# homenc/HElib

Hardware: NVIDIA H100
Metric: ctxt_mults_per_s (higher is better)
Workload: dtype u64

## Files before the change

helib_b200/csrc/hb_device_v1.cuh:

```cuda
#pragma once
#include <utility>
#include "hb_device.cuh"

#define HB1_RS 17
#define HB1_BS 273

__device__ __forceinline__ void hb_group_sync(int group, int nthreads) {
#ifdef HB_SIM
  cusim::bar_sync(1 + group, nthreads);
#else
  asm volatile("bar.sync %0, %1;" ::"r"(1 + group), "r"(nthreads) : "memory");
#endif
}

__device__ __forceinline__ void hb1_mac128(u64& hi, u64& lo, u64 a, u64 b) {
#ifdef HB_SIM
  hb_mac128(hi, lo, a, b);
#else
  asm("{\n\t.reg .u64 pl, ph;\n\t"
      "mul.lo.u64 pl, %2, %3;\n\t"
      "mul.hi.u64 ph, %2, %3;\n\t"
      "add.cc.u64 %0, %0, pl;\n\t"
      "addc.u64 %1, %1, ph;\n\t}"
      : "+l"(lo), "+l"(hi)
// ... 137 lines not shown
  asm volatile("cp.async.ca.shared.global [%0], [%1], 8;" ::"r"(sa), "l"(src) : "memory");
#endif
}
__device__ __forceinline__ void hb1_cp_commit() {
#ifndef HB_SIM
  asm volatile("cp.async.commit_group;" ::: "memory");
#endif
}
template <int N> __device__ __forceinline__ void hb1_cp_wait() {
#ifndef HB_SIM
  asm volatile("cp.async.wait_group %0;" ::"n"(N) : "memory");
#endif
}

#define HB1_STAGE (16 * HB1_BS + 8)

struct Hb1Unit { int rowi, ug, it; };
__device__ __forceinline__ Hb1Unit hb1_unit_next(Hb1Unit x, int G, int nitems) {
  if (++x.it == nitems) { x.it = 0; if (++x.ug == G) { x.ug = 0; ++x.rowi; } }
  return x;
}
__device__ __forceinline__ Hb1Unit hb1_unit(long u, int G, int nitems) {
  Hb1Unit x;
  const unsigned per_row = (unsigned)(G * nitems), uu = (unsigned)u;
  x.rowi = (int)(uu / per_row);
  const int rem = (int)(uu - (unsigned)x.rowi * per_row);
  x.ug = rem / nitems;
  x.it = rem - x.ug * nitems;
  return x;
}

template <bool SP>
__global__ void __launch_bounds__(256, 2) k1_fwd_blk(const HbPrimeDev* __restrict__ primes, const HB_GRID_CONSTANT Hb1BlkJob J) {
  HB_SMEM_DECL
  u64* S = HB_SMEM;
  u64* O = S + 2 * HB1_STAGE;
  ulonglong2* TW1 = (ulonglong2*)(O + 16 * 256);
  const int tid = threadIdx.x;
  const int n1 = J.logN - 8;
  const int G = 1 << (n1 - 4);
  const long U = (long)J.rows.n * G * J.nitems;
  const long ubeg = U * blockIdx.x / gridDim.x, uend = U * (blockIdx.x + 1) / gridDim.x;
  if (ubeg >= uend) return;
  const int blk1 = tid >> 4, lo = tid & 15;
  const int hi = tid >> 4, blk2 = tid & 15;
  const unsigned hrev = hb1_brev4(hi);
  const bool epi1 = J.epi == 1, epi3 = J.epi == 3, lazy = J.lazy != 0;
  const int own = blk1 * HB1_BS + lo;
  Hb1TwPtr tw1;
  tw1.p[0] = TW1 + blk1 * 16; tw1.p[1] = tw1.p[0] + 1; tw1.p[2] = tw1.p[0] + 3; tw1.p[3] = tw1.p[0] + 7;

  auto src_ptr = [&](const Hb1Unit& x) {
    const unsigned b = hb_brev((x.ug << 4) + blk1, n1);
    return J.src[x.it] + ((size_t)J.rows.prime[x.rowi] << J.logN) + ((size_t)b << 8) + lo;
  };
  Hb1Unit cur = hb1_unit(ubeg, G, J.nitems);
  {
    const u64* src = src_ptr(cur);
    hb1_unroll<16>([&](auto r) { hb1_cp8(S + own + HB1_RS * r, src + 16 * r); });
  }
  hb1_cp_commit();
  int key = -1, buf = 0;
  u64 q = 0, sc = 0, sc_s = 0;
  Hb1Mod M; M.nq = 0; M.qb = 0; M.qb2 = 0; M.qt = 0; M.qsh = 0;
  Hb1TwReg tw2;
  for (long u = ubeg; u < uend; u++, buf ^= 1) {
    if (cur.rowi * G + cur.ug != key) {
      key = cur.rowi * G + cur.ug;
      const HbPrimeDev P = primes[J.rows.prime[cur.rowi]];
      q = P.q; M.nq = P.nq; M.qb = P.qb; M.qb2 = P.qb + P.qb; M.qt = P.qt; M.qsh = P.qsh;
      sc = J.scal[cur.rowi]; sc_s = J.scal_s[cur.rowi];
      const unsigned b1 = hb_brev((cur.ug << 4) + blk1, n1), b2 = hb_brev((cur.ug << 4) + blk2, n1);
      if (lo < 15) {
        int e = lo, k = e >= 7 ? 3 : (e >= 3 ? 2 : (e >= 1 ? 1 : 0));
        int g = e - ((1 << k) - 1);
        TW1[blk1 * 16 + e] = P.fw[((size_t)1 << (n1 + k)) + ((size_t)b1 << k) + g];
      }
      tw2.load([&](int k, int g) { return P.fw[((size_t)1 << (n1 + 4 + k)) + ((size_t)b2 << (4 + k)) + ((size_t)hi << k) + g]; });
      __syncthreads();
    }
    u64* Sb = S + buf * HB1_STAGE;
    const size_t doff = ((size_t)J.rows.prime[cur.rowi] << J.logN) + (cur.ug << 4) + blk2;
    u64* dst = J.dst[cur.it] + doff;
    const bool epi = epi1 || (epi3 && sc != 0);
    u64* old = epi3 ? J.dst2[cur.it] + doff : dst;
    if (epi) {
      hb1_unroll<16>([&](auto l) { hb1_cp8(O + l * 256 + tid, old + ((size_t)((hb1_brev4(l) << 4) | hrev) << n1)); });
    }
    hb1_cp_commit();
    Hb1Unit nxt = cur;
    if (u + 1 < uend) {
      nxt = hb1_unit_next(cur, G, J.nitems);
      const u64* src = src_ptr(nxt);
      u64* Sn = S + (buf ^ 1) * HB1_STAGE;
      hb1_unroll<16>([&](auto r) { hb1_cp8(Sn + own + HB1_RS * r, src + 16 * r); });
    }
    hb1_cp_commit();
    hb1_cp_wait<2>();
    u64 a[16];
    hb1_unroll<16>([&](auto r) { a[r] = Sb[own + HB1_RS * r]; });
    hb1_r16_fwd<SP>(a, tw1, M);
    hb1_unroll<16>([&](auto r) { Sb[own + HB1_RS * r] = a[r]; });
    __syncthreads();
    hb1_unroll<16>([&](auto l) { a[l] = Sb[blk2 * HB1_BS + HB1_RS * hi + l]; });
    hb1_r16_fwd<SP>(a, tw2, M);
    hb1_cp_wait<1>();
    hb1_unroll<16>([&](auto l) {
      const size_t o = (size_t)((hb1_brev4(l) << 4) | hrev) << n1;
      if (epi) {
        u64 v = hb1_shoup4<SP>(O[l * 256 + tid] - a[l] + (M.qb2 + M.qb), sc, sc_s, M);
        if (!lazy) v = hb1_canon4(v, q);
        old[o] = v;
      }
      if (!epi1) dst[o] = lazy ? a[l] : hb1_canon_fwd(a[l], q, M.qb);
    });
    __syncthreads();
    cur = nxt;
  }
  hb1_cp_wait<0>();
}

template <bool SP>
__global__ void __launch_bounds__(256, 1) k1_fwd_blk_tensor(const HbPrimeDev* __restrict__ primes, const HB_GRID_CONSTANT Hb1BlkJob J) {
  HB_SMEM_DECL
  u64* S = HB_SMEM;
  u64* O = S + 2 * HB1_STAGE;
  ulonglong2* TW1 = (ulonglong2*)(O + 16 * 256);
  u64* V = (u64*)(TW1 + 256);
  const int tid = threadIdx.x;
  const int n1 = J.logN - 8;
  const int G = 1 << (n1 - 4);
  const long U = (long)J.rows.n * G * J.nitems;
  const long ubeg = U * blockIdx.x / gridDim.x, uend = U * (blockIdx.x + 1) / gridDim.x;
  if (ubeg >= uend) return;
  const int blk1 = tid >> 4, lo = tid & 15;
  const int hi = tid >> 4, blk2 = tid & 15;
  const unsigned hrev = hb1_brev4(hi);
  const int own = blk1 * HB1_BS + lo;
  u64* const Vt = V + tid;
  Hb1TwPtr tw1;
  tw1.p[0] = TW1 + blk1 * 16; tw1.p[1] = tw1.p[0] + 1; tw1.p[2] = tw1.p[0] + 3; tw1.p[3] = tw1.p[0] + 7;

  auto prefetch = [&](u64* Sn, const Hb1Unit& x, int k) {
    const unsigned b = hb_brev((x.ug << 4) + blk1, n1);
    const u64* src = J.src[4 * x.it + k] + ((size_t)J.rows.prime[x.rowi] << J.logN) + ((size_t)b << 8) + lo;
    hb1_unroll<16>([&](auto r) { hb1_cp8(Sn + own + HB1_RS * r, src + 16 * r); });
  };
  Hb1Unit cur = hb1_unit(ubeg, G, J.nitems);
  prefetch(S, cur, 0);
  hb1_cp_commit();
  int key = -1;
  u64 q = 0, sc = 0, sc_s = 0, c64 = 0, c64_s = 0, one_s = 0;
  Hb1Mod M; M.nq = 0; M.qb = 0; M.qb2 = 0; M.qt = 0; M.qsh = 0;
  Hb1TwReg tw2;
  for (long u = ubeg; u < uend; u++) {
    if (cur.rowi * G + cur.ug != key) {
      key = cur.rowi * G + cur.ug;
      const HbPrimeDev P = primes[J.rows.prime[cur.rowi]];
      q = P.q; M.nq = P.nq; M.qb = P.qb; M.qb2 = P.qb + P.qb; M.qt = P.qt; M.qsh = P.qsh;
      c64 = P.c64; c64_s = P.c64_s; one_s = P.one_s;
      sc = J.scal[cur.rowi]; sc_s = J.scal_s[cur.rowi];
      const unsigned b1 = hb_brev((cur.ug << 4) + blk1, n1), b2 = hb_brev((cur.ug << 4) + blk2, n1);
      if (lo < 15) {
        int e = lo, k = e >= 7 ? 3 : (e >= 3 ? 2 : (e >= 1 ? 1 : 0));
        int g = e - ((1 << k) - 1);
        TW1[blk1 * 16 + e] = P.fw[((size_t)1 << (n1 + k)) + ((size_t)b1 << k) + g];
      }
      tw2.load([&](int k, int g) { return P.fw[((size_t)1 << (n1 + 4 + k)) + ((size_t)b2 << (4 + k)) + ((size_t)hi << k) + g]; });
      __syncthreads();
    }
    const size_t doff = ((size_t)J.rows.prime[cur.rowi] << J.logN) + (cur.ug << 4) + blk2;
    u64* const* dst = J.dst + 4 * cur.it;
    const bool more = u + 1 < uend;
    const Hb1Unit nxt = more ? hb1_unit_next(cur, G, J.nitems) : cur;
#pragma unroll 1
    for (int k = 0; k < 4; k++) {
      u64* Sb = S + (k & 1) * HB1_STAGE;
      const u64* old = dst[k] + doff;
      hb1_unroll<16>([&](auto l) { hb1_cp8(O + l * 256 + tid, old + ((size_t)((hb1_brev4(l) << 4) | hrev) << n1)); });
      hb1_cp_commit();
      if (k < 3) prefetch(S + ((k + 1) & 1) * HB1_STAGE, cur, k + 1);
      else if (more) prefetch(S, nxt, 0);
      hb1_cp_commit();
      hb1_cp_wait<2>();
      u64 a[16];
      hb1_unroll<16>([&](auto r) { a[r] = Sb[own + HB1_RS * r]; });
      hb1_r16_fwd<SP>(a, tw1, M);
      hb1_unroll<16>([&](auto r) { Sb[own + HB1_RS * r] = a[r]; });
      __syncthreads();
      hb1_unroll<16>([&](auto l) { a[l] = Sb[blk2 * HB1_BS + HB1_RS * hi + l]; });
      hb1_r16_fwd<SP>(a, tw2, M);
      hb1_cp_wait<1>();
      hb1_unroll<16>([&](auto l) {
        a[l] = hb1_shoup4<SP>(O[l * 256 + tid] - a[l] + (M.qb2 + M.qb), sc, sc_s, M);
      });
      if (k < 2) {
        hb1_unroll<16>([&](auto l) { Vt[k * 4096 + l * 256] = a[l]; });
      } else if (k == 2) {
        hb1_unroll<16>([&](auto l) {
          const size_t o = doff + ((size_t)((hb1_brev4(l) << 4) | hrev) << n1);
          const u64 x0 = Vt[l * 256], x1 = Vt[4096 + l * 256], v = a[l];
          dst[0][o] = hb_reduce128(__umul64hi(x0, v), x0 * v, q, c64, c64_s, one_s);
          Vt[2 * 4096 + l * 256] = hb_reduce128(__umul64hi(x1, v), x1 * v, q, c64, c64_s, one_s);
        });
      } else {
        hb1_unroll<16>([&](auto l) {
          const size_t o = doff + ((size_t)((hb1_brev4(l) << 4) | hrev) << n1);
          const u64 x0 = Vt[l * 256], x1 = Vt[4096 + l * 256], v = a[l];
          u64 h = 0, w = Vt[2 * 4096 + l * 256];
          hb1_mac128(h, w, x0, v);
          dst[1][o] = hb_reduce128(h, w, q, c64, c64_s, one_s);
          dst[2][o] = hb_reduce128(__umul64hi(x1, v), x1 * v, q, c64, c64_s, one_s);
          dst[3][o] = v;
        });
      }
      __syncthreads();
    }
    cur = nxt;
  }
  hb1_cp_wait<0>();
}

template <bool SP>
__global__ void __launch_bounds__(256, 2) k1_inv_blk(const HbPrimeDev* __restrict__ primes, const HB_GRID_CONSTANT Hb1BlkJob J) {
  HB_SMEM_DECL
  u64* S = HB_SMEM;
  ulonglong2* TW1 = (ulonglong2*)(S + 2 * HB1_STAGE);
  const int tid = threadIdx.x;
  const int n1 = J.logN - 8;
  const int G = 1 << (n1 - 4);
  const long U = (long)J.rows.n * G * J.nitems;
  const long ubeg = U * blockIdx.x / gridDim.x, uend = U * (blockIdx.x + 1) / gridDim.x;
  if (ubeg >= uend) return;
  const int blk1 = tid >> 4, lo = tid & 15;
  const int hi = tid >> 4, blk2 = tid & 15;
  const unsigned hrev = hb1_brev4(hi);
  Hb1TwPtr tw1;
  tw1.p[0] = TW1 + blk1 * 16; tw1.p[1] = tw1.p[0] + 1; tw1.p[2] = tw1.p[0] + 3; tw1.p[3] = tw1.p[0] + 7;
  const int own = blk2 * HB1_BS + HB1_RS * hi;
  auto src_ptr = [&](const Hb1Unit& x) {
    return J.src[x.it] + ((size_t)J.rows.prime[x.rowi] << J.logN) + (x.ug << 4) + blk2;
  };
  Hb1Unit cur = hb1_unit(ubeg, G, J.nitems);
  {
    const u64* src = src_ptr(cur);
    hb1_unroll<16>([&](auto l) { hb1_cp8(S + own + l, src + ((size_t)((hb1_brev4(l) << 4) | hrev) << n1)); });
  }
  hb1_cp_commit();
  int key = -1, buf = 0;
  u64 q = 0;
  Hb1Mod M; M.nq = 0; M.qb = 0; M.qb2 = 0; M.qt = 0; M.qsh = 0;
  unsigned b1 = 0;
  Hb1TwReg tw2;
  for (long u = ubeg; u < uend; u++, buf ^= 1) {
    if (cur.rowi * G + cur.ug != key) {
      key = cur.rowi * G + cur.ug;
      const HbPrimeDev P = primes[J.rows.prime[cur.rowi]];
      q = P.q; M.nq = P.nq; M.qb = P.qb; M.qb2 = P.qb + P.qb; M.qt = P.qt; M.qsh = P.qsh;
      b1 = hb_brev((cur.ug << 4) + blk1, n1);
      const unsigned b2 = hb_brev((cur.ug << 4) + blk2, n1);
      if (lo < 15) {
        int e = lo, k = e >= 7 ? 3 : (e >= 3 ? 2 : (e >= 1 ? 1 : 0));
        int g = e - ((1 << k) - 1);
        TW1[blk1 * 16 + e] = P.iw[((size_t)1 << (n1 + k)) + ((size_t)b1 << k) + g];
      }
      tw2.load([&](int k, int g) { return P.iw[((size_t)1 << (n1 + 4 + k)) + ((size_t)b2 << (4 + k)) + ((size_t)hi << k) + g]; });
      __syncthreads();
    }
    u64* Sb = S + buf * HB1_STAGE;
    Hb1Unit nxt = cur;
    if (u + 1 < uend) {
      nxt = hb1_unit_next(cur, G, J.nitems);
      const u64* src = src_ptr(nxt);
      u64* Sn = S + (buf ^ 1) * HB1_STAGE;
      hb1_unroll<16>([&](auto l) { hb1_cp8(Sn + own + l, src + ((size_t)((hb1_brev4(l) << 4) | hrev) << n1)); });
    }
    hb1_cp_commit();
    hb1_cp_wait<1>();
    u64 a[16];
    hb1_unroll<16>([&](auto l) { a[l] = Sb[own + l]; });
    hb1_r16_inv<SP>(a, tw2, M);
    hb1_unroll<16>([&](auto l) { Sb[own + l] = a[l]; });
    __syncthreads();
    hb1_unroll<16>([&](auto r) { a[r] = Sb[blk1 * HB1_BS + HB1_RS * r + lo]; });
    hb1_r16_inv<SP>(a, tw1, M);
    u64* dst = J.dst[cur.it] + ((size_t)J.rows.prime[cur.rowi] << J.logN) + ((size_t)b1 << 8) + lo;
    hb1_unroll<16>([&](auto r) { dst[16 * r] = J.epi == 2 ? a[r] : hb1_canon_inv(a[r], q); });
    __syncthreads();
    cur = nxt;
  }
  hb1_cp_wait<0>();
}

struct Hb1ColsJob {
  int logN;
  HbRows rows;
  int nitems;
  const u64* src[HB_MAXB];
  u64* dst[HB_MAXB];
  int has_scal, npeers;
  u64 scal[HB_MAXROWS], scal_s[HB_MAXROWS];
  u64* peer[8][HB_MAXB];
};

// ... 316 lines not shown
```

helib_b200/csrc/hb_engine.cu:

```cuda
#include "hb_device.cuh"
#include "hb_device_v1.cuh"
#include "hb_device_v2.cuh"
#include "hb_device_gen.cuh"
#include "hb_device_prg.cuh"

#include <algorithm>
#include <cmath>
#include <cstdarg>
#include <cstdio>
#include <cstdlib>
#include <cstring>
#include <map>
#include <set>
#include <string>
#include <vector>

#include "../../include/helib_b200.h"

typedef unsigned __int128 u128;

static size_t blk_tensor_smem() {
  return (2 * HB1_STAGE + 16 * 256 + 3 * 16 * 256) * sizeof(u64) + 256 * sizeof(ulonglong2);
}

static thread_local char g_err[512] = "";
static thread_local int g_chunk = HB_MAXB;
static int hb_fail(int code, const char* fmt, ...) {
  va_list ap; va_start(ap, fmt); vsnprintf(g_err, sizeof(g_err), fmt, ap); va_end(ap);
  return code;
}
#define HB_CUDA(x) do { cudaError_t e_ = (x); if (e_ != cudaSuccess) return hb_fail(HB_ERR_CUDA, "%s failed: %s (%s:%d)", #x, cudaGetErrorString(e_), __FILE__, __LINE__); } while (0)
#define HB_TRY(x) do { int r_ = (x); if (r_ != HB_OK) return r_; } while (0)

static inline u64 h_mulmod(u64 a, u64 b, u64 q) { return (u64)((u128)a * b % q); }
static inline u64 h_powmod(u64 a, u64 e, u64 q) {
  u64 r = 1 % q; a %= q;
  while (e) { if (e & 1) r = h_mulmod(r, a, q); a = h_mulmod(a, a, q); e >>= 1; }
  return r;
// ... 200 lines not shown
      u64 qi = c->q[i];
      HbPrimeDev& P = c->h_primes[i];
      memset(&P, 0, sizeof(P));
      P.q = qi; P.c64 = (u64)(((u128)1 << 64) % qi); P.c64_s = h_shoup(P.c64, qi); P.one_s = (u64)(((u128)1 << 64) / qi);
      P.nq = 0 - qi; P.qb = 4 * qi;
      { int sh = 0; u64 t = qi - 1; while ((t & 1) == 0) { t >>= 1; sh++; }
        if (sh >= 32 && t < (1ULL << 32)) { P.qt = (unsigned)t; P.qsh = (unsigned)(sh - 32); } }
    }
    HB_TRY(ctx_alloc(c, (void**)&c->d_primes, sizeof(HbPrimeDev) * nprimes));
    HB_CUDA(cudaMemcpy(c->d_primes, c->h_primes.data(), sizeof(HbPrimeDev) * nprimes, cudaMemcpyHostToDevice));
    HB_TRY(ctx_alloc(c, (void**)&c->d_stats, 4 * sizeof(u64)));
    HB_CUDA(cudaMemset(c->d_stats, 0, 4 * sizeof(u64)));
#ifndef HB_SIM
    HB_CUDA(cudaFuncSetAttribute(k_fwd_blk, cudaFuncAttributeMaxDynamicSharedMemorySize, 64 * 1024));
    HB_CUDA(cudaFuncSetAttribute(k_inv_blk, cudaFuncAttributeMaxDynamicSharedMemorySize, 64 * 1024));
    HB_CUDA(cudaFuncSetAttribute(k1_fwd_blk<true>, cudaFuncAttributeMaxDynamicSharedMemorySize, 112 * 1024));
  HB_CUDA(cudaFuncSetAttribute(k1_fwd_blk<false>, cudaFuncAttributeMaxDynamicSharedMemorySize, 112 * 1024));
    HB_CUDA(cudaFuncSetAttribute(k1_inv_blk<true>, cudaFuncAttributeMaxDynamicSharedMemorySize, 80 * 1024));
  HB_CUDA(cudaFuncSetAttribute(k1_inv_blk<false>, cudaFuncAttributeMaxDynamicSharedMemorySize, 80 * 1024));
    HB_CUDA(cudaFuncSetAttribute(k2_fwd_blk<true>, cudaFuncAttributeMaxDynamicSharedMemorySize, (int)HB2_SMEM_BYTES));
    HB_CUDA(cudaFuncSetAttribute(k2_fwd_blk<false>, cudaFuncAttributeMaxDynamicSharedMemorySize, (int)HB2_SMEM_BYTES));
    HB_CUDA(cudaFuncSetAttribute(k2_inv_blk<true>, cudaFuncAttributeMaxDynamicSharedMemorySize, (int)HB2_SMEM_BYTES));
    HB_CUDA(cudaFuncSetAttribute(k2_inv_blk<false>, cudaFuncAttributeMaxDynamicSharedMemorySize, (int)HB2_SMEM_BYTES));
#endif
    HB_TRY(gen_init(c, psi));
    *out = c;
    return HB_OK;
  }
  std::vector<ulonglong2> tw((size_t)nprimes * 2 * N);
  std::vector<u64> pw(N);
  std::vector<unsigned> brev(N);
  for (size_t k = 0; k < N; k++) { unsigned r = 0; for (int b = 0; b < c->logN; b++) if (k >> b & 1) r |= 1u << (c->logN - 1 - b); brev[k] = r; }
  HB_TRY(ctx_alloc(c, (void**)&c->d_tw, tw.size() * sizeof(ulonglong2)));
  c->h_primes.resize(nprimes);
// ... 22 lines not shown
  HB_CUDA(cudaMemcpy(c->d_primes, c->h_primes.data(), sizeof(HbPrimeDev) * nprimes, cudaMemcpyHostToDevice));
  HB_TRY(ctx_alloc(c, (void**)&c->d_stats, 4 * sizeof(u64)));
  HB_CUDA(cudaMemset(c->d_stats, 0, 4 * sizeof(u64)));
#ifndef HB_SIM
  HB_CUDA(cudaFuncSetAttribute(k_conv, cudaFuncAttributeMaxDynamicSharedMemorySize, (int)c->max_smem + 1024));
  HB_CUDA(cudaFuncSetAttribute(k_fwd_blk, cudaFuncAttributeMaxDynamicSharedMemorySize, 64 * 1024));
  HB_CUDA(cudaFuncSetAttribute(k_inv_blk, cudaFuncAttributeMaxDynamicSharedMemorySize, 64 * 1024));
  HB_CUDA(cudaFuncSetAttribute(k2_fwd_blk<true>, cudaFuncAttributeMaxDynamicSharedMemorySize, (int)HB2_SMEM_BYTES));
  HB_CUDA(cudaFuncSetAttribute(k2_fwd_blk<false>, cudaFuncAttributeMaxDynamicSharedMemorySize, (int)HB2_SMEM_BYTES));
  HB_CUDA(cudaFuncSetAttribute(k2_inv_blk<true>, cudaFuncAttributeMaxDynamicSharedMemorySize, (int)HB2_SMEM_BYTES));
  HB_CUDA(cudaFuncSetAttribute(k2_inv_blk<false>, cudaFuncAttributeMaxDynamicSharedMemorySize, (int)HB2_SMEM_BYTES));
  HB_CUDA(cudaFuncSetAttribute(k1_conv1<true>, cudaFuncAttributeMaxDynamicSharedMemorySize, 128 * 1024));
  HB_CUDA(cudaFuncSetAttribute(k1_conv1<false>, cudaFuncAttributeMaxDynamicSharedMemorySize, 128 * 1024));
  HB_CUDA(cudaFuncSetAttribute(k1_conv<true>, cudaFuncAttributeMaxDynamicSharedMemorySize, 227 * 1024));
  HB_CUDA(cudaFuncSetAttribute(k1_conv<false>, cudaFuncAttributeMaxDynamicSharedMemorySize, 227 * 1024));
  HB_CUDA(cudaFuncSetAttribute(k1_fwd_blk<true>, cudaFuncAttributeMaxDynamicSharedMemorySize, 112 * 1024));
  HB_CUDA(cudaFuncSetAttribute(k1_fwd_blk<false>, cudaFuncAttributeMaxDynamicSharedMemorySize, 112 * 1024));
  HB_CUDA(cudaFuncSetAttribute(k1_inv_blk<true>, cudaFuncAttributeMaxDynamicSharedMemorySize, 80 * 1024));
  HB_CUDA(cudaFuncSetAttribute(k1_inv_blk<false>, cudaFuncAttributeMaxDynamicSharedMemorySize, 80 * 1024));
  HB_CUDA(cudaFuncSetAttribute(k1_fwd_blk_tensor<true>, cudaFuncAttributeMaxDynamicSharedMemorySize, (int)blk_tensor_smem()));
  HB_CUDA(cudaFuncSetAttribute(k1_fwd_blk_tensor<false>, cudaFuncAttributeMaxDynamicSharedMemorySize, (int)blk_tensor_smem()));
#endif
  *out = c;
  return HB_OK;
}

extern "C" void hb_ctx_destroy(hb_ctx* c) {
  if (!c) return;
  if (c->stream) cudaStreamSynchronize(c->stream);
  for (auto& kv : c->convs) { cudaFree(kv.second.blob); cudaFree(kv.second.d); }
  for (hb_poly* p : c->pool) { cudaFree(p->d); delete p; }
  cudaFree(c->pw.d_cube_to_poly); cudaFree(c->pw.d_short_to_long); cudaFree(c->pw.cube); cudaFree(c->pw.rows);
  cudaFree(c->d_frac); cudaFree(c->d_z); cudaFree(c->d_max); cudaFree(c->d_bcast);
  cudaFree(c->gen.d_rep); cudaFree(c->gen.d_irep); cudaFree(c->gen.d_gp); cudaFree(c->gen.d_primes_cyc); cudaFree(c->gen.d_primes_cyc2); cudaFree(c->gen.tab);
  cudaFree(c->gen.d_W);
  cudaFree(c->gen.w0); cudaFree(c->gen.w1); cudaFree(c->gen.wt); cudaFree(c->gen.cA); cudaFree(c->gen.cB);
// ... 437 lines not shown
static bool v1_cols_ok(hb_ctx* c) { return !c->force_v0 && c->log_blk == 8 && c->logN - 8 == 8; }
static int pick_item_groups(hb_ctx* c, long ctas_per_item_group, int nitems) {
  int best = 1; double best_eff = -1;
  for (int z = 1; z <= nitems; z++) {
    long ctas = ctas_per_item_group * z;
    long waves = (ctas + c->resident_ctas - 1) / c->resident_ctas;
    int per = (nitems + z - 1) / z;
    double eff = (double)ctas / (double)(waves * c->resident_ctas) * ((double)nitems / (double)(per * z));
    if (eff > best_eff + 0.02) { best_eff = eff; best = z; }
  }
  return best;
}
static int launch_blk_v1(hb_ctx* c, int dir, const u64* const* src, u64* const* dst, int nitems, const int32_t* idx, int n,
                         int epi, const u64* scal, int lazy = 0, u64* const* dst2 = nullptr) {
  const int n1 = c->logN - 8;
  const size_t smem = (2 * HB1_STAGE + (dir > 0 ? 16 * 256 : 0)) * sizeof(u64) + 256 * sizeof(ulonglong2);
  for (int r0 = 0; r0 < n; r0 += HB_MAXROWS) {
    int nr = std::min(HB_MAXROWS, n - r0);
    Hb1BlkJob J; memset(&J, 0, sizeof(J));
    J.logN = c->logN; J.epi = epi; J.lazy = lazy;
    if (dir < 0) J.epi = v1_cols_ok(c) ? 2 : 0;
    fill_rows(J.rows, idx + r0, nr);
    for (int i = 0; i < nr; i++) if (scal) { J.scal[i] = scal[r0 + i]; J.scal_s[i] = h_shoup(scal[r0 + i], c->q[idx[r0 + i]]); }
    J.nitems = nitems;
    for (int i = 0; i < nitems; i++) { J.src[i] = src[i]; J.dst[i] = dst[i]; if (dst2) J.dst2[i] = dst2[i]; }
    long units = (long)nr * nitems << (n1 - 4);
    dim3 grid((unsigned)std::min<long>(units, c->resident_ctas));
    pre_launch(c);
    const bool sp = all_special(c);
    if (dir > 0) { if (sp) HB_LAUNCH(k1_fwd_blk<true>, grid, dim3(256), smem, c->stream, c->d_primes, J); else HB_LAUNCH(k1_fwd_blk<false>, grid, dim3(256), smem, c->stream, c->d_primes, J); HB_TRY(post_launch(c, epi == 1 ? "k1_fwd_blk_subscale" : (epi == 3 ? "k1_fwd_blk_digits" : "k1_fwd_blk"), (u64)(epi == 1 ? 3 : 2) * nr * nitems * c->N * 8)); }
    else { if (sp) HB_LAUNCH(k1_inv_blk<true>, grid, dim3(256), smem, c->stream, c->d_primes, J); else HB_LAUNCH(k1_inv_blk<false>, grid, dim3(256), smem, c->stream, c->d_primes, J); HB_TRY(post_launch(c, "k1_inv_blk", (u64)2 * nr * nitems * c->N * 8)); }
  }
  return HB_OK;
}
static int launch_blk_tensor_v1(hb_ctx* c, const u64* const* src, u64* const* dst, int nitems, const int32_t* idx, int n, const u64* scal) {
  const int n1 = c->logN - 8;
  for (int r0 = 0; r0 < n; r0 += HB_MAXROWS) {
    int nr = std::min(HB_MAXROWS, n - r0);
    Hb1BlkJob J; memset(&J, 0, sizeof(J));
    J.logN = c->logN; J.epi = 1; J.lazy = 1;
    fill_rows(J.rows, idx + r0, nr);
    for (int i = 0; i < nr; i++) { J.scal[i] = scal[r0 + i]; J.scal_s[i] = h_shoup(scal[r0 + i], c->q[idx[r0 + i]]); }
    J.nitems = nitems;
    for (int i = 0; i < 4 * nitems; i++) { J.src[i] = src[i]; J.dst[i] = dst[i]; }
    long units = (long)nr * nitems << (n1 - 4);
    dim3 grid((unsigned)std::min<long>(units, std::max(1, c->resident_ctas / 2)));
    pre_launch(c);
    if (all_special(c)) HB_LAUNCH(k1_fwd_blk_tensor<true>, grid, dim3(256), blk_tensor_smem(), c->stream, c->d_primes, J);
    else HB_LAUNCH(k1_fwd_blk_tensor<false>, grid, dim3(256), blk_tensor_smem(), c->stream, c->d_primes, J);
    HB_TRY(post_launch(c, "k1_fwd_blk_tensor", (u64)12 * nr * nitems * c->N * 8));
  }
  return HB_OK;
}

#define HB_TMAP_SLAB 512
#ifndef HB_SIM
typedef CUresult (*hb_encode_tiled_fn)(CUtensorMap*, CUtensorMapDataType, cuuint32_t, void*, const cuuint64_t*, const cuuint64_t*,
                                       const cuuint32_t*, const cuuint32_t*, CUtensorMapInterleave, CUtensorMapSwizzle,
                                       CUtensorMapL2promotion, CUtensorMapFloatOOBfill);
static hb_encode_tiled_fn hb_encode_tiled() {
  static hb_encode_tiled_fn fn = [] {
    void* p = nullptr; cudaDriverEntryPointQueryResult qr;
    if (cudaGetDriverEntryPoint("cuTensorMapEncodeTiled", &p, cudaEnableDefault, &qr) != cudaSuccess || qr != cudaDriverEntryPointSuccess) p = nullptr;
    return (hb_encode_tiled_fn)p;
// ... 1959 lines not shown
```

Before: 2948.

## Deepen NTT block kernel pipelines to triple-buffered inputs with prefetched epilogue operands

The forward and inverse blocked NTT kernels move from double to triple buffering of staged input tiles, and the forward kernel also double-buffers the epilogue's old-value tile so it is fetched one unit ahead. The tensor kernel prefetches its per-part epilogue operands after the previous part's stores instead of right before use. To fit the extra shared memory, launch bounds drop to one CTA per SM and the grid is halved, which trades occupancy for deeper async-copy overlap. The change also adds compile-time ablation switches and a standalone microbenchmark.

```diff
diff --git a/bench_micro/ubench_blk.cu b/bench_micro/ubench_blk.cu
--- /dev/null
+++ b/bench_micro/ubench_blk.cu
@@ -0,0 +1,106 @@
+#include <cstdio>
+#include <cstdlib>
+#include <cstring>
+#include <vector>
+#include <cuda_runtime.h>
+#include "../helib_b200/csrc/hb_device_v1.cuh"
+
+#define CK(x) do { cudaError_t e_ = (x); if (e_ != cudaSuccess) { fprintf(stderr, "%s: %s (line %d)\n", #x, cudaGetErrorString(e_), __LINE__); exit(1); } } while (0)
+
+typedef unsigned __int128 u128;
+static const int LOGN = 16, NPR = 30, NPOLY = 192;
+static const size_t N = (size_t)1 << LOGN;
+
+static u64 rng_state = 0x9E3779B97F4A7C15ULL;
+static u64 rnd() { rng_state ^= rng_state << 13; rng_state ^= rng_state >> 7; rng_state ^= rng_state << 17; return rng_state; }
+
+__global__ void fill_random(u64* p, size_t n, u64 q, u64 seed) {
+  for (size_t i = blockIdx.x * (size_t)blockDim.x + threadIdx.x; i < n; i += (size_t)gridDim.x * blockDim.x) {
+    u64 x = (i + 1) * 0x9E3779B97F4A7C15ULL ^ seed;
+    x ^= x >> 29; x *= 0xBF58476D1CE4E5B9ULL; x ^= x >> 32;
+    p[i] = x % q;
+  }
+}
+
+struct Primes { HbPrimeDev* d; std::vector<u64> q; };
+static Primes make_primes(bool sp, ulonglong2* tw) {
+  Primes P; std::vector<HbPrimeDev> h(NPR);
+  std::vector<ulonglong2> t(2 * N);
+  for (int i = 0; i < NPR; i++) {
+    const u64 qt = (1ULL << 27) - 2 * i - 1;
+    const u64 q = sp ? (qt << 33) + 1 : (1ULL << 60) - (((u64)i + 1) << 20) - 1;
+    P.q.push_back(q);
+    HbPrimeDev& H = h[i]; memset(&H, 0, sizeof(H));
+    H.q = q; H.c64 = (u64)(((u128)1 << 64) % q); H.c64_s = (u64)(((u128)H.c64 << 64) / q); H.one_s = (u64)(((u128)1 << 64) / q);
+    H.nq = 0 - q; H.qb = 4 * q;
+    if (sp) { H.qt = (unsigned)qt; H.qsh = 1; }
+    for (size_t k = 0; k < 2 * N; k++) { u64 w = rnd() % q; t[k] = make_ulonglong2(w, (u64)(((u128)w << 64) / q)); }
+    CK(cudaMemcpy(tw + (size_t)i * 2 * N, t.data(), t.size() * sizeof(ulonglong2), cudaMemcpyHostToDevice));
+    H.fw = tw + (size_t)i * 2 * N; H.iw = H.fw + N;
+  }
+  CK(cudaMalloc(&P.d, sizeof(HbPrimeDev) * NPR));
+  CK(cudaMemcpy(P.d, h.data(), sizeof(HbPrimeDev) * NPR, cudaMemcpyHostToDevice));
+  return P;
+}
+
+int main() {
+  int nsm = 0; CK(cudaDeviceGetAttribute(&nsm, cudaDevAttrMultiProcessorCount, 0));
+  cudaDeviceProp prop; CK(cudaGetDeviceProperties(&prop, 0));
+  const int ctas = HB1_BLK_CTAS_PER_SM * nsm;
+  printf("# %s, %d SMs, %d CTAs, ablation: noglobal %d nopass2 %d noepi %d\n", prop.name, nsm, ctas, HB1_ABL_NOGLOBAL, HB1_ABL_NOPASS2, HB1_ABL_NOEPI);
+  ulonglong2* tw; CK(cudaMalloc(&tw, sizeof(ulonglong2) * 2 * N * NPR));
+  std::vector<u64*> poly(NPOLY);
+  for (auto& p : poly) CK(cudaMalloc(&p, sizeof(u64) * N * NPR));
+  for (int sp = 1; sp >= 0; sp--) {
+    Primes P = make_primes(sp != 0, tw);
+    for (int i = 0; i < NPOLY; i++) fill_random<<<528, 256>>>(poly[i], N * NPR, P.q[0], 1234567 + i);
+    CK(cudaDeviceSynchronize());
+#define SET_SMEM(K, B) CK(cudaFuncSetAttribute(K, cudaFuncAttributeMaxDynamicSharedMemorySize, (int)(B)))
+    SET_SMEM(k1_fwd_blk<true>, HB1_FWD_SMEM); SET_SMEM(k1_fwd_blk<false>, HB1_FWD_SMEM);
+    SET_SMEM(k1_inv_blk<true>, HB1_INV_SMEM); SET_SMEM(k1_inv_blk<false>, HB1_INV_SMEM);
+    SET_SMEM(k1_fwd_blk_tensor<true>, HB1_TENSOR_SMEM); SET_SMEM(k1_fwd_blk_tensor<false>, HB1_TENSOR_SMEM);
+    struct Case { const char* name; int kind, epi, lazy, rows, items, nscal; };
+    const Case cases[] = {{"fwd_plain", 0, 0, 0, 19, 64, 0}, {"fwd_subscale", 0, 1, 0, 19, 64, 19}, {"fwd_digits", 0, 3, 1, 19, 32, 9},
+                          {"inv", 1, 2, 0, 10, 64, 0}, {"tensor", 2, 1, 1, 19, 16, 19}};
+    for (const Case& C : cases) {
+      static Hb1BlkJob J; memset(&J, 0, sizeof(J));
+      J.logN = LOGN; J.epi = C.epi; J.lazy = C.lazy; J.nitems = C.items;
+      J.rows.n = C.rows;
+      for (int r = 0; r < C.rows; r++) {
+        J.rows.prime[r] = r;
+        const u64 q = P.q[r], s = r < C.nscal ? rnd() % q : 0;
+        J.scal[r] = s; J.scal_s[r] = (u64)(((u128)s << 64) / q);
+      }
+      const int nptr = C.kind == 2 ? 4 * C.items : C.items;
+      for (int i = 0; i < nptr; i++) { J.src[i] = poly[i]; J.dst[i] = poly[64 + i]; J.dst2[i] = poly[128 + i]; }
+      const long units = (long)C.rows * C.items * (N >> 12);
+      const long g = C.kind == 2 ? nsm : ctas;
+      const dim3 grid((unsigned)(units < g ? units : g));
+      auto launch = [&]() {
+        if (C.kind == 0) { if (sp) k1_fwd_blk<true><<<grid, 256, HB1_FWD_SMEM>>>(P.d, J); else k1_fwd_blk<false><<<grid, 256, HB1_FWD_SMEM>>>(P.d, J); }
+        else if (C.kind == 1) { if (sp) k1_inv_blk<true><<<grid, 256, HB1_INV_SMEM>>>(P.d, J); else k1_inv_blk<false><<<grid, 256, HB1_INV_SMEM>>>(P.d, J); }
+        else { if (sp) k1_fwd_blk_tensor<true><<<grid, 256, HB1_TENSOR_SMEM>>>(P.d, J); else k1_fwd_blk_tensor<false><<<grid, 256, HB1_TENSOR_SMEM>>>(P.d, J); }
+      };
+      for (int w = 0; w < 3; w++) launch();
+      CK(cudaGetLastError()); CK(cudaDeviceSynchronize());
+      cudaEvent_t e0, e1; CK(cudaEventCreate(&e0)); CK(cudaEventCreate(&e1));
+      const int reps = 20;
+      CK(cudaEventRecord(e0));
+      for (int i = 0; i < reps; i++) launch();
+      CK(cudaEventRecord(e1)); CK(cudaEventSynchronize(e1)); CK(cudaGetLastError());
+      float ms; CK(cudaEventElapsedTime(&ms, e0, e1)); ms /= reps;
+      const int parts = C.kind == 2 ? 4 : 1;
+      const double bfly = (double)parts * C.rows * C.items * (N / 2) * 8;
+      double rowmoves = C.kind == 2 ? 12.0 * C.rows : (C.epi == 1 ? 3.0 * C.rows : 2.0 * C.rows + (C.epi == 3 ? 2.0 * C.nscal : 0));
+      if (HB1_ABL_NOEPI && C.kind != 1) rowmoves = C.kind == 2 ? 8.0 * C.rows : 2.0 * C.rows;
+      const double bytes = HB1_ABL_NOGLOBAL ? 0.0 : rowmoves * C.items * N * 8;
+      printf("%-13s %-7s rows %2d items %2d: %8.4f ms  %.3e butterflies/s  %7.1f GB/s\n", C.name, sp ? "shift" : "generic", C.rows, C.items,
+             ms, bfly / (ms * 1e-3), bytes / (ms * 1e-3) / 1e9);
+      CK(cudaEventDestroy(e0)); CK(cudaEventDestroy(e1));
+    }
+    CK(cudaFree(P.d));
+  }
+  for (auto p : poly) CK(cudaFree(p));
+  CK(cudaFree(tw));
+  return 0;
+}
diff --git a/helib_b200/csrc/hb_device_v1.cuh b/helib_b200/csrc/hb_device_v1.cuh
--- a/helib_b200/csrc/hb_device_v1.cuh
+++ b/helib_b200/csrc/hb_device_v1.cuh
@@ -4,6 +4,16 @@
 
 #define HB1_RS 17
 #define HB1_BS 273
+
+#ifndef HB1_ABL_NOGLOBAL
+#define HB1_ABL_NOGLOBAL 0
+#endif
+#ifndef HB1_ABL_NOPASS2
+#define HB1_ABL_NOPASS2 0
+#endif
+#ifndef HB1_ABL_NOEPI
+#define HB1_ABL_NOEPI 0
+#endif
 
 __device__ __forceinline__ void hb_group_sync(int group, int nthreads) {
 #ifdef HB_SIM
@@ -175,6 +185,10 @@
 }
 
 #define HB1_STAGE (16 * HB1_BS + 8)
+#define HB1_FWD_SMEM ((3 * HB1_STAGE + 2 * 16 * 256) * 8 + 256 * 16)
+#define HB1_INV_SMEM (3 * HB1_STAGE * 8 + 256 * 16)
+#define HB1_TENSOR_SMEM ((2 * HB1_STAGE + 16 * 256 + 3 * 16 * 256) * 8 + 256 * 16)
+#define HB1_BLK_CTAS_PER_SM 1
 
 struct Hb1Unit { int rowi, ug, it; };
 __device__ __forceinline__ Hb1Unit hb1_unit_next(Hb1Unit x, int G, int nitems) {
@@ -192,17 +206,18 @@
 }
 
 template <bool SP>
-__global__ void __launch_bounds__(256, 2) k1_fwd_blk(const HbPrimeDev* __restrict__ primes, const HB_GRID_CONSTANT Hb1BlkJob J) {
+__global__ void __launch_bounds__(256, 1) k1_fwd_blk(const HbPrimeDev* __restrict__ primes, const HB_GRID_CONSTANT Hb1BlkJob J) {
   HB_SMEM_DECL
   u64* S = HB_SMEM;
-  u64* O = S + 2 * HB1_STAGE;
-  ulonglong2* TW1 = (ulonglong2*)(O + 16 * 256);
+  u64* O = S + 3 * HB1_STAGE;
+  ulonglong2* TW1 = (ulonglong2*)(O + 2 * 16 * 256);
   const int tid = threadIdx.x;
   const int n1 = J.logN - 8;
   const int G = 1 << (n1 - 4);
   const long U = (long)J.rows.n * G * J.nitems;
   const long ubeg = U * blockIdx.x / gridDim.x, uend = U * (blockIdx.x + 1) / gridDim.x;
   if (ubeg >= uend) return;
+  const long nu = uend - ubeg;
   const int blk1 = tid >> 4, lo = tid & 15;
   const int hi = tid >> 4, blk2 = tid & 15;
   const unsigned hrev = hb1_brev4(hi);
@@ -211,21 +226,33 @@
   Hb1TwPtr tw1;
   tw1.p[0] = TW1 + blk1 * 16; tw1.p[1] = tw1.p[0] + 1; tw1.p[2] = tw1.p[0] + 3; tw1.p[3] = tw1.p[0] + 7;
 
-  auto src_ptr = [&](const Hb1Unit& x) {
+  auto stage_in = [&](u64* Sn, const Hb1Unit& x) {
     const unsigned b = hb_brev((x.ug << 4) + blk1, n1);
-    return J.src[x.it] + ((size_t)J.rows.prime[x.rowi] << J.logN) + ((size_t)b << 8) + lo;
+    const u64* src = J.src[x.it] + ((size_t)J.rows.prime[x.rowi] << J.logN) + ((size_t)b << 8) + lo;
+    if (!HB1_ABL_NOGLOBAL) hb1_unroll<16>([&](auto r) { hb1_cp8(Sn + own + HB1_RS * r, src + 16 * r); });
+  };
+  auto has_epi = [&](const Hb1Unit& x) { return !HB1_ABL_NOEPI && (epi1 || (epi3 && J.scal[x.rowi] != 0)); };
+  auto dst_off = [&](const Hb1Unit& x) { return ((size_t)J.rows.prime[x.rowi] << J.logN) + (x.ug << 4) + blk2; };
+  auto old_ptr = [&](const Hb1Unit& x) { return (epi3 ? J.dst2[x.it] : J.dst[x.it]) + dst_off(x); };
+  auto stage_old = [&](u64* On, const Hb1Unit& x) {
+    const u64* old = old_ptr(x);
+    if (!HB1_ABL_NOGLOBAL && has_epi(x))
+      hb1_unroll<16>([&](auto l) { hb1_cp8(On + l * 256 + tid, old + ((size_t)((hb1_brev4(l) << 4) | hrev) << n1)); });
   };
   Hb1Unit cur = hb1_unit(ubeg, G, J.nitems);
-  {
-    const u64* src = src_ptr(cur);
-    hb1_unroll<16>([&](auto r) { hb1_cp8(S + own + HB1_RS * r, src + 16 * r); });
-  }
+  Hb1Unit nx1 = hb1_unit_next(cur, G, J.nitems), nx2 = hb1_unit_next(nx1, G, J.nitems);
+  stage_in(S, cur);
   hb1_cp_commit();
-  int key = -1, buf = 0;
+  hb1_cp_commit();
+  if (nu > 1) stage_in(S + HB1_STAGE, nx1);
+  hb1_cp_commit();
+  stage_old(O, cur);
+  hb1_cp_commit();
+  int key = -1, sb = 0;
   u64 q = 0, sc = 0, sc_s = 0;
   Hb1Mod M; M.nq = 0; M.qb = 0; M.qb2 = 0; M.qt = 0; M.qsh = 0;
   Hb1TwReg tw2;
-  for (long u = ubeg; u < uend; u++, buf ^= 1) {
+  for (long i = 0; i < nu; i++) {
     if (cur.rowi * G + cur.ug != key) {
       key = cur.rowi * G + cur.ug;
       const HbPrimeDev P = primes[J.rows.prime[cur.rowi]];
@@ -240,43 +267,42 @@
       tw2.load([&](int k, int g) { return P.fw[((size_t)1 << (n1 + 4 + k)) + ((size_t)b2 << (4 + k)) + ((size_t)hi << k) + g]; });
       __syncthreads();
     }
-    u64* Sb = S + buf * HB1_STAGE;
-    const size_t doff = ((size_t)J.rows.prime[cur.rowi] << J.logN) + (cur.ug << 4) + blk2;
-    u64* dst = J.dst[cur.it] + doff;
-    const bool epi = epi1 || (epi3 && sc != 0);
-    u64* old = epi3 ? J.dst2[cur.it] + doff : dst;
-    if (epi) {
-      hb1_unroll<16>([&](auto l) { hb1_cp8(O + l * 256 + tid, old + ((size_t)((hb1_brev4(l) << 4) | hrev) << n1)); });
-    }
+    if (i + 2 < nu) stage_in(S + (sb == 0 ? 2 : sb - 1) * HB1_STAGE, nx2);
     hb1_cp_commit();
-    Hb1Unit nxt = cur;
-    if (u + 1 < uend) {
-      nxt = hb1_unit_next(cur, G, J.nitems);
-      const u64* src = src_ptr(nxt);
-      u64* Sn = S + (buf ^ 1) * HB1_STAGE;
-      hb1_unroll<16>([&](auto r) { hb1_cp8(Sn + own + HB1_RS * r, src + 16 * r); });
-    }
+    if (i + 1 < nu) stage_old(O + ((i + 1) & 1) * 16 * 256, nx1);
     hb1_cp_commit();
-    hb1_cp_wait<2>();
+    u64* Sb = S + sb * HB1_STAGE;
+    const u64* Ob = O + (i & 1) * 16 * 256;
+    hb1_cp_wait<5>();
     u64 a[16];
     hb1_unroll<16>([&](auto r) { a[r] = Sb[own + HB1_RS * r]; });
     hb1_r16_fwd<SP>(a, tw1, M);
     hb1_unroll<16>([&](auto r) { Sb[own + HB1_RS * r] = a[r]; });
     __syncthreads();
     hb1_unroll<16>([&](auto l) { a[l] = Sb[blk2 * HB1_BS + HB1_RS * hi + l]; });
-    hb1_r16_fwd<SP>(a, tw2, M);
-    hb1_cp_wait<1>();
-    hb1_unroll<16>([&](auto l) {
-      const size_t o = (size_t)((hb1_brev4(l) << 4) | hrev) << n1;
-      if (epi) {
-        u64 v = hb1_shoup4<SP>(O[l * 256 + tid] - a[l] + (M.qb2 + M.qb), sc, sc_s, M);
+    if (!HB1_ABL_NOPASS2) hb1_r16_fwd<SP>(a, tw2, M);
+    hb1_cp_wait<2>();
+    const bool epi = has_epi(cur);
+    u64* dst = J.dst[cur.it] + dst_off(cur);
+    u64* old = old_ptr(cur);
+    auto put_x = [&](size_t o, int l) {
+      const u64 x = lazy ? a[l] : hb1_canon_fwd(a[l], q, M.qb);
+      if (HB1_ABL_NOGLOBAL) Sb[own + HB1_RS * l] ^= x; else dst[o] = x;
+    };
+    if (epi) {
+      hb1_unroll<16>([&](auto l) {
+        const size_t o = (size_t)((hb1_brev4(l) << 4) | hrev) << n1;
+        u64 v = hb1_shoup4<SP>(Ob[l * 256 + tid] - a[l] + (M.qb2 + M.qb), sc, sc_s, M);
         if (!lazy) v = hb1_canon4(v, q);
-        old[o] = v;
-      }
-      if (!epi1) dst[o] = lazy ? a[l] : hb1_canon_fwd(a[l], q, M.qb);
-    });
+        if (HB1_ABL_NOGLOBAL) Sb[own + HB1_RS * l] ^= v; else old[o] = v;
+        if (!epi1) put_x(o, l);
+      });
+    } else {
+      hb1_unroll<16>([&](auto l) { put_x((size_t)((hb1_brev4(l) << 4) | hrev) << n1, l); });
+    }
     __syncthreads();
-    cur = nxt;
+    cur = nx1; nx1 = nx2; nx2 = hb1_unit_next(nx2, G, J.nitems);
+    sb = sb == 2 ? 0 : sb + 1;
   }
   hb1_cp_wait<0>();
 }
@@ -305,10 +331,18 @@
   auto prefetch = [&](u64* Sn, const Hb1Unit& x, int k) {
     const unsigned b = hb_brev((x.ug << 4) + blk1, n1);
     const u64* src = J.src[4 * x.it + k] + ((size_t)J.rows.prime[x.rowi] << J.logN) + ((size_t)b << 8) + lo;
-    hb1_unroll<16>([&](auto r) { hb1_cp8(Sn + own + HB1_RS * r, src + 16 * r); });
+    if (!HB1_ABL_NOGLOBAL) hb1_unroll<16>([&](auto r) { hb1_cp8(Sn + own + HB1_RS * r, src + 16 * r); });
+  };
+  auto dst_off = [&](const Hb1Unit& x) { return ((size_t)J.rows.prime[x.rowi] << J.logN) + (x.ug << 4) + blk2; };
+  auto stage_old = [&](const Hb1Unit& x, int k) {
+    const u64* old = J.dst[4 * x.it + k] + dst_off(x);
+    if (!HB1_ABL_NOGLOBAL && !HB1_ABL_NOEPI)
+      hb1_unroll<16>([&](auto l) { hb1_cp8(O + l * 256 + tid, old + ((size_t)((hb1_brev4(l) << 4) | hrev) << n1)); });
   };
   Hb1Unit cur = hb1_unit(ubeg, G, J.nitems);
   prefetch(S, cur, 0);
+  hb1_cp_commit();
+  stage_old(cur, 0);
   hb1_cp_commit();
   int key = -1;
   u64 q = 0, sc = 0, sc_s = 0, c64 = 0, c64_s = 0, one_s = 0;
@@ -330,16 +364,13 @@
       tw2.load([&](int k, int g) { return P.fw[((size_t)1 << (n1 + 4 + k)) + ((size_t)b2 << (4 + k)) + ((size_t)hi << k) + g]; });
       __syncthreads();
     }
-    const size_t doff = ((size_t)J.rows.prime[cur.rowi] << J.logN) + (cur.ug << 4) + blk2;
+    const size_t doff = dst_off(cur);
     u64* const* dst = J.dst + 4 * cur.it;
     const bool more = u + 1 < uend;
     const Hb1Unit nxt = more ? hb1_unit_next(cur, G, J.nitems) : cur;
 #pragma unroll 1
     for (int k = 0; k < 4; k++) {
       u64* Sb = S + (k & 1) * HB1_STAGE;
-      const u64* old = dst[k] + doff;
-      hb1_unroll<16>([&](auto l) { hb1_cp8(O + l * 256 + tid, old + ((size_t)((hb1_brev4(l) << 4) | hrev) << n1)); });
-      hb1_cp_commit();
       if (k < 3) prefetch(S + ((k + 1) & 1) * HB1_STAGE, cur, k + 1);
       else if (more) prefetch(S, nxt, 0);
       hb1_cp_commit();
@@ -350,18 +381,19 @@
       hb1_unroll<16>([&](auto r) { Sb[own + HB1_RS * r] = a[r]; });
       __syncthreads();
       hb1_unroll<16>([&](auto l) { a[l] = Sb[blk2 * HB1_BS + HB1_RS * hi + l]; });
-      hb1_r16_fwd<SP>(a, tw2, M);
+      if (!HB1_ABL_NOPASS2) hb1_r16_fwd<SP>(a, tw2, M);
       hb1_cp_wait<1>();
       hb1_unroll<16>([&](auto l) {
-        a[l] = hb1_shoup4<SP>(O[l * 256 + tid] - a[l] + (M.qb2 + M.qb), sc, sc_s, M);
+        if (!HB1_ABL_NOEPI) a[l] = hb1_shoup4<SP>(O[l * 256 + tid] - a[l] + (M.qb2 + M.qb), sc, sc_s, M);
       });
+      auto put = [&](u64* d, size_t o, int l, u64 v) { if (HB1_ABL_NOGLOBAL) Sb[own + HB1_RS * l] ^= v; else d[o] = v; };
       if (k < 2) {
         hb1_unroll<16>([&](auto l) { Vt[k * 4096 + l * 256] = a[l]; });
       } else if (k == 2) {
         hb1_unroll<16>([&](auto l) {
           const size_t o = doff + ((size_t)((hb1_brev4(l) << 4) | hrev) << n1);
           const u64 x0 = Vt[l * 256], x1 = Vt[4096 + l * 256], v = a[l];
-          dst[0][o] = hb_reduce128(__umul64hi(x0, v), x0 * v, q, c64, c64_s, one_s);
+          put(dst[0], o, l, hb_reduce128(__umul64hi(x0, v), x0 * v, q, c64, c64_s, one_s));
           Vt[2 * 4096 + l * 256] = hb_reduce128(__umul64hi(x1, v), x1 * v, q, c64, c64_s, one_s);
         });
       } else {
@@ -370,11 +402,14 @@
           const u64 x0 = Vt[l * 256], x1 = Vt[4096 + l * 256], v = a[l];
           u64 h = 0, w = Vt[2 * 4096 + l * 256];
           hb1_mac128(h, w, x0, v);
-          dst[1][o] = hb_reduce128(h, w, q, c64, c64_s, one_s);
-          dst[2][o] = hb_reduce128(__umul64hi(x1, v), x1 * v, q, c64, c64_s, one_s);
-          dst[3][o] = v;
+          put(dst[1], o, l, hb_reduce128(h, w, q, c64, c64_s, one_s));
+          put(dst[2], o, l, hb_reduce128(__umul64hi(x1, v), x1 * v, q, c64, c64_s, one_s));
+          put(dst[3], o, l, v);
         });
       }
+      if (k < 3) stage_old(cur, k + 1);
+      else if (more) stage_old(nxt, 0);
+      hb1_cp_commit();
       __syncthreads();
     }
     cur = nxt;
@@ -383,37 +418,39 @@
 }
 
 template <bool SP>
-__global__ void __launch_bounds__(256, 2) k1_inv_blk(const HbPrimeDev* __restrict__ primes, const HB_GRID_CONSTANT Hb1BlkJob J) {
+__global__ void __launch_bounds__(256, 1) k1_inv_blk(const HbPrimeDev* __restrict__ primes, const HB_GRID_CONSTANT Hb1BlkJob J) {
   HB_SMEM_DECL
   u64* S = HB_SMEM;
-  ulonglong2* TW1 = (ulonglong2*)(S + 2 * HB1_STAGE);
+  ulonglong2* TW1 = (ulonglong2*)(S + 3 * HB1_STAGE);
   const int tid = threadIdx.x;
   const int n1 = J.logN - 8;
   const int G = 1 << (n1 - 4);
   const long U = (long)J.rows.n * G * J.nitems;
   const long ubeg = U * blockIdx.x / gridDim.x, uend = U * (blockIdx.x + 1) / gridDim.x;
   if (ubeg >= uend) return;
+  const long nu = uend - ubeg;
   const int blk1 = tid >> 4, lo = tid & 15;
   const int hi = tid >> 4, blk2 = tid & 15;
   const unsigned hrev = hb1_brev4(hi);
   Hb1TwPtr tw1;
   tw1.p[0] = TW1 + blk1 * 16; tw1.p[1] = tw1.p[0] + 1; tw1.p[2] = tw1.p[0] + 3; tw1.p[3] = tw1.p[0] + 7;
   const int own = blk2 * HB1_BS + HB1_RS * hi;
-  auto src_ptr = [&](const Hb1Unit& x) {
-    return J.src[x.it] + ((size_t)J.rows.prime[x.rowi] << J.logN) + (x.ug << 4) + blk2;
+  auto stage_in = [&](u64* Sn, const Hb1Unit& x) {
+    const u64* src = J.src[x.it] + ((size_t)J.rows.prime[x.rowi] << J.logN) + (x.ug << 4) + blk2;
+    if (!HB1_ABL_NOGLOBAL) hb1_unroll<16>([&](auto l) { hb1_cp8(Sn + own + l, src + ((size_t)((hb1_brev4(l) << 4) | hrev) << n1)); });
   };
   Hb1Unit cur = hb1_unit(ubeg, G, J.nitems);
-  {
-    const u64* src = src_ptr(cur);
-    hb1_unroll<16>([&](auto l) { hb1_cp8(S + own + l, src + ((size_t)((hb1_brev4(l) << 4) | hrev) << n1)); });
-  }
+  Hb1Unit nx1 = hb1_unit_next(cur, G, J.nitems), nx2 = hb1_unit_next(nx1, G, J.nitems);
+  stage_in(S, cur);
   hb1_cp_commit();
-  int key = -1, buf = 0;
+  if (nu > 1) stage_in(S + HB1_STAGE, nx1);
+  hb1_cp_commit();
+  int key = -1, sb = 0;
   u64 q = 0;
   Hb1Mod M; M.nq = 0; M.qb = 0; M.qb2 = 0; M.qt = 0; M.qsh = 0;
   unsigned b1 = 0;
   Hb1TwReg tw2;
-  for (long u = ubeg; u < uend; u++, buf ^= 1) {
+  for (long i = 0; i < nu; i++) {
     if (cur.rowi * G + cur.ug != key) {
       key = cur.rowi * G + cur.ug;
       const HbPrimeDev P = primes[J.rows.prime[cur.rowi]];
@@ -428,27 +465,25 @@
       tw2.load([&](int k, int g) { return P.iw[((size_t)1 << (n1 + 4 + k)) + ((size_t)b2 << (4 + k)) + ((size_t)hi << k) + g]; });
       __syncthreads();
     }
-    u64* Sb = S + buf * HB1_STAGE;
-    Hb1Unit nxt = cur;
-    if (u + 1 < uend) {
-      nxt = hb1_unit_next(cur, G, J.nitems);
-      const u64* src = src_ptr(nxt);
-      u64* Sn = S + (buf ^ 1) * HB1_STAGE;
-      hb1_unroll<16>([&](auto l) { hb1_cp8(Sn + own + l, src + ((size_t)((hb1_brev4(l) << 4) | hrev) << n1)); });
-    }
+    if (i + 2 < nu) stage_in(S + (sb == 0 ? 2 : sb - 1) * HB1_STAGE, nx2);
     hb1_cp_commit();
-    hb1_cp_wait<1>();
+    u64* Sb = S + sb * HB1_STAGE;
+    hb1_cp_wait<2>();
     u64 a[16];
     hb1_unroll<16>([&](auto l) { a[l] = Sb[own + l]; });
     hb1_r16_inv<SP>(a, tw2, M);
     hb1_unroll<16>([&](auto l) { Sb[own + l] = a[l]; });
     __syncthreads();
     hb1_unroll<16>([&](auto r) { a[r] = Sb[blk1 * HB1_BS + HB1_RS * r + lo]; });
-    hb1_r16_inv<SP>(a, tw1, M);
+    if (!HB1_ABL_NOPASS2) hb1_r16_inv<SP>(a, tw1, M);
     u64* dst = J.dst[cur.it] + ((size_t)J.rows.prime[cur.rowi] << J.logN) + ((size_t)b1 << 8) + lo;
-    hb1_unroll<16>([&](auto r) { dst[16 * r] = J.epi == 2 ? a[r] : hb1_canon_inv(a[r], q); });
+    hb1_unroll<16>([&](auto r) {
+      const u64 x = J.epi == 2 ? a[r] : hb1_canon_inv(a[r], q);
+      if (HB1_ABL_NOGLOBAL) Sb[blk1 * HB1_BS + HB1_RS * r + lo] ^= x; else dst[16 * r] = x;
+    });
     __syncthreads();
-    cur = nxt;
+    cur = nx1; nx1 = nx2; nx2 = hb1_unit_next(nx2, G, J.nitems);
+    sb = sb == 2 ? 0 : sb + 1;
   }
   hb1_cp_wait<0>();
 }
diff --git a/helib_b200/csrc/hb_engine.cu b/helib_b200/csrc/hb_engine.cu
--- a/helib_b200/csrc/hb_engine.cu
+++ b/helib_b200/csrc/hb_engine.cu
@@ -18,10 +18,6 @@
 #include "../../include/helib_b200.h"
 
 typedef unsigned __int128 u128;
-
-static size_t blk_tensor_smem() {
-  return (2 * HB1_STAGE + 16 * 256 + 3 * 16 * 256) * sizeof(u64) + 256 * sizeof(ulonglong2);
-}
 
 static thread_local char g_err[512] = "";
 static thread_local int g_chunk = HB_MAXB;
@@ -252,10 +248,10 @@
 #ifndef HB_SIM
     HB_CUDA(cudaFuncSetAttribute(k_fwd_blk, cudaFuncAttributeMaxDynamicSharedMemorySize, 64 * 1024));
     HB_CUDA(cudaFuncSetAttribute(k_inv_blk, cudaFuncAttributeMaxDynamicSharedMemorySize, 64 * 1024));
-    HB_CUDA(cudaFuncSetAttribute(k1_fwd_blk<true>, cudaFuncAttributeMaxDynamicSharedMemorySize, 112 * 1024));
-  HB_CUDA(cudaFuncSetAttribute(k1_fwd_blk<false>, cudaFuncAttributeMaxDynamicSharedMemorySize, 112 * 1024));
-    HB_CUDA(cudaFuncSetAttribute(k1_inv_blk<true>, cudaFuncAttributeMaxDynamicSharedMemorySize, 80 * 1024));
-  HB_CUDA(cudaFuncSetAttribute(k1_inv_blk<false>, cudaFuncAttributeMaxDynamicSharedMemorySize, 80 * 1024));
+    HB_CUDA(cudaFuncSetAttribute(k1_fwd_blk<true>, cudaFuncAttributeMaxDynamicSharedMemorySize, HB1_FWD_SMEM));
+    HB_CUDA(cudaFuncSetAttribute(k1_fwd_blk<false>, cudaFuncAttributeMaxDynamicSharedMemorySize, HB1_FWD_SMEM));
+    HB_CUDA(cudaFuncSetAttribute(k1_inv_blk<true>, cudaFuncAttributeMaxDynamicSharedMemorySize, HB1_INV_SMEM));
+    HB_CUDA(cudaFuncSetAttribute(k1_inv_blk<false>, cudaFuncAttributeMaxDynamicSharedMemorySize, HB1_INV_SMEM));
     HB_CUDA(cudaFuncSetAttribute(k2_fwd_blk<true>, cudaFuncAttributeMaxDynamicSharedMemorySize, (int)HB2_SMEM_BYTES));
     HB_CUDA(cudaFuncSetAttribute(k2_fwd_blk<false>, cudaFuncAttributeMaxDynamicSharedMemorySize, (int)HB2_SMEM_BYTES));
     HB_CUDA(cudaFuncSetAttribute(k2_inv_blk<true>, cudaFuncAttributeMaxDynamicSharedMemorySize, (int)HB2_SMEM_BYTES));
@@ -308,12 +304,12 @@
   HB_CUDA(cudaFuncSetAttribute(k1_conv1<false>, cudaFuncAttributeMaxDynamicSharedMemorySize, 128 * 1024));
   HB_CUDA(cudaFuncSetAttribute(k1_conv<true>, cudaFuncAttributeMaxDynamicSharedMemorySize, 227 * 1024));
   HB_CUDA(cudaFuncSetAttribute(k1_conv<false>, cudaFuncAttributeMaxDynamicSharedMemorySize, 227 * 1024));
-  HB_CUDA(cudaFuncSetAttribute(k1_fwd_blk<true>, cudaFuncAttributeMaxDynamicSharedMemorySize, 112 * 1024));
-  HB_CUDA(cudaFuncSetAttribute(k1_fwd_blk<false>, cudaFuncAttributeMaxDynamicSharedMemorySize, 112 * 1024));
-  HB_CUDA(cudaFuncSetAttribute(k1_inv_blk<true>, cudaFuncAttributeMaxDynamicSharedMemorySize, 80 * 1024));
-  HB_CUDA(cudaFuncSetAttribute(k1_inv_blk<false>, cudaFuncAttributeMaxDynamicSharedMemorySize, 80 * 1024));
-  HB_CUDA(cudaFuncSetAttribute(k1_fwd_blk_tensor<true>, cudaFuncAttributeMaxDynamicSharedMemorySize, (int)blk_tensor_smem()));
-  HB_CUDA(cudaFuncSetAttribute(k1_fwd_blk_tensor<false>, cudaFuncAttributeMaxDynamicSharedMemorySize, (int)blk_tensor_smem()));
+  HB_CUDA(cudaFuncSetAttribute(k1_fwd_blk<true>, cudaFuncAttributeMaxDynamicSharedMemorySize, HB1_FWD_SMEM));
+  HB_CUDA(cudaFuncSetAttribute(k1_fwd_blk<false>, cudaFuncAttributeMaxDynamicSharedMemorySize, HB1_FWD_SMEM));
+  HB_CUDA(cudaFuncSetAttribute(k1_inv_blk<true>, cudaFuncAttributeMaxDynamicSharedMemorySize, HB1_INV_SMEM));
+  HB_CUDA(cudaFuncSetAttribute(k1_inv_blk<false>, cudaFuncAttributeMaxDynamicSharedMemorySize, HB1_INV_SMEM));
+  HB_CUDA(cudaFuncSetAttribute(k1_fwd_blk_tensor<true>, cudaFuncAttributeMaxDynamicSharedMemorySize, HB1_TENSOR_SMEM));
+  HB_CUDA(cudaFuncSetAttribute(k1_fwd_blk_tensor<false>, cudaFuncAttributeMaxDynamicSharedMemorySize, HB1_TENSOR_SMEM));
 #endif
   *out = c;
   return HB_OK;
@@ -781,7 +777,7 @@
 static int launch_blk_v1(hb_ctx* c, int dir, const u64* const* src, u64* const* dst, int nitems, const int32_t* idx, int n,
                          int epi, const u64* scal, int lazy = 0, u64* const* dst2 = nullptr) {
   const int n1 = c->logN - 8;
-  const size_t smem = (2 * HB1_STAGE + (dir > 0 ? 16 * 256 : 0)) * sizeof(u64) + 256 * sizeof(ulonglong2);
+  const size_t smem = dir > 0 ? HB1_FWD_SMEM : HB1_INV_SMEM;
   for (int r0 = 0; r0 < n; r0 += HB_MAXROWS) {
     int nr = std::min(HB_MAXROWS, n - r0);
     Hb1BlkJob J; memset(&J, 0, sizeof(J));
@@ -792,7 +788,7 @@
     J.nitems = nitems;
     for (int i = 0; i < nitems; i++) { J.src[i] = src[i]; J.dst[i] = dst[i]; if (dst2) J.dst2[i] = dst2[i]; }
     long units = (long)nr * nitems << (n1 - 4);
-    dim3 grid((unsigned)std::min<long>(units, c->resident_ctas));
+    dim3 grid((unsigned)std::min<long>(units, std::max(1, c->resident_ctas / 2)));
     pre_launch(c);
     const bool sp = all_special(c);
     if (dir > 0) { if (sp) HB_LAUNCH(k1_fwd_blk<true>, grid, dim3(256), smem, c->stream, c->d_primes, J); else HB_LAUNCH(k1_fwd_blk<false>, grid, dim3(256), smem, c->stream, c->d_primes, J); HB_TRY(post_launch(c, epi == 1 ? "k1_fwd_blk_subscale" : (epi == 3 ? "k1_fwd_blk_digits" : "k1_fwd_blk"), (u64)(epi == 1 ? 3 : 2) * nr * nitems * c->N * 8)); }
@@ -813,8 +809,8 @@
     long units = (long)nr * nitems << (n1 - 4);
     dim3 grid((unsigned)std::min<long>(units, std::max(1, c->resident_ctas / 2)));
     pre_launch(c);
-    if (all_special(c)) HB_LAUNCH(k1_fwd_blk_tensor<true>, grid, dim3(256), blk_tensor_smem(), c->stream, c->d_primes, J);
-    else HB_LAUNCH(k1_fwd_blk_tensor<false>, grid, dim3(256), blk_tensor_smem(), c->stream, c->d_primes, J);
+    if (all_special(c)) HB_LAUNCH(k1_fwd_blk_tensor<true>, grid, dim3(256), HB1_TENSOR_SMEM, c->stream, c->d_primes, J);
+    else HB_LAUNCH(k1_fwd_blk_tensor<false>, grid, dim3(256), HB1_TENSOR_SMEM, c->stream, c->d_primes, J);
     HB_TRY(post_launch(c, "k1_fwd_blk_tensor", (u64)12 * nr * nitems * c->N * 8));
   }
   return HB_OK;
```

New measurement: 3087 (median of 6 runs). +4.7%, better.
